# BattleZips/BattleZips-Halo2

Measured on AMD Instinct MI355X. Metric: complete proofs per second (synthesis + create_proof), BoardCircuit, k=14, IPA/Pasta, higher is better.
Workload: dtype u32x8 (255-bit modular integer, Montgomery)

## Files before the change

battlezips-halo2_amd/csrc/ctx.hpp:

```cpp
#pragma once
#include <hip/hip_runtime.h>
#include <sched.h>

#include <algorithm>
#include <cstdint>
#include <cstdlib>
#include <cstring>
#include <mutex>
#include <string>
#include <vector>

#include "../../include/bzh2.h"

struct bzh_bases {
    int curve = 0;
    size_t n = 0;
    uint32_t* d_xy = nullptr;
    int device = 0;
    int pre_c = 0;
    int pre_nwin = 0;
    size_t row_stride = 0;
    size_t vec_col_stride = 0;
    uint32_t* d_xy29 = nullptr;
};
// ... 91 lines not shown
    if ((al & 15) == 0) {
        const size_t n16 = bytes / 16;
        const unsigned blocks = (unsigned)std::min<size_t>((n16 + 255) / 256, 2048);
        hipLaunchKernelGGL(k_xfer16, dim3(blocks), dim3(256), 0, ctx->stream, (uint4*)dst, (const uint4*)src, n16);
    } else if ((al & 3) == 0) {
        const size_t n4 = bytes / 4;
        const unsigned blocks = (unsigned)std::min<size_t>((n4 + 255) / 256, 2048);
        hipLaunchKernelGGL(k_xfer4, dim3(blocks), dim3(256), 0, ctx->stream, (uint32_t*)dst, (const uint32_t*)src, n4);
    } else {
        BZH_HIP_TRY(ctx, hipMemcpyAsync(dst, src, bytes, fallback, ctx->stream));
        return BZH_OK;
    }
    BZH_HIP_TRY(ctx, hipGetLastError());
    return BZH_OK;
}
inline int pin_big_ensure(bzh_ctx* ctx, size_t bytes) {
    if (ctx->pin_big_bytes >= bytes) return BZH_OK;
    BZH_HIP_TRY(ctx, hipStreamSynchronize(ctx->stream));
    for (auto& p : ctx->pending_d2h) memcpy(p.dst, p.slot, p.bytes);
    ctx->pending_d2h.clear();
    if (ctx->pin_big) BZH_HIP_TRY(ctx, hipHostFree(ctx->pin_big));
    ctx->pin_big = nullptr;
    ctx->pin_big_bytes = 0;
    const size_t want = bytes + (bytes >> 2) + 4096;
    BZH_HIP_TRY(ctx, hipHostMalloc((void**)&ctx->pin_big, want, hipHostMallocDefault));
    ctx->pin_big_bytes = want;
    ctx->pin_big_off = 0;
    return BZH_OK;
}
inline int pin_big_take(bzh_ctx* ctx, size_t bytes, char** out) {
// ... 54 lines not shown
    return bytes > ((size_t)1 << 20) ? pin_big_take(ctx, bytes, slot) : pin_ring_take(ctx, bytes, slot);
}
inline int h2d_commit(bzh_ctx* ctx, void* dst, const char* slot, size_t bytes) {
    return xfer_launch(ctx, dst, slot, bytes, hipMemcpyHostToDevice);
}
inline int d2h_async(bzh_ctx* ctx, void* host_dst, const void* dev_src, size_t bytes) {
    if (!bytes) return BZH_OK;
    char* slot = nullptr;
    int rc = bytes > ((size_t)1 << 20) ? pin_big_take(ctx, bytes, &slot) : pin_ring_take(ctx, bytes, &slot);
    if (rc) return rc;
    rc = xfer_launch(ctx, slot, dev_src, bytes, hipMemcpyDeviceToHost);
    if (rc) return rc;
    ctx->pending_d2h.push_back({host_dst, slot, bytes});
    return BZH_OK;
}
inline int d2h_finish(bzh_ctx* ctx) {
    BZH_HIP_TRY(ctx, hipStreamSynchronize(ctx->stream));
    for (auto& p : ctx->pending_d2h) memcpy(p.dst, p.slot, p.bytes);
    ctx->pending_d2h.clear();
    return BZH_OK;
}

struct ScopedTimer {
    bzh_ctx* ctx;
    int cls;
    hipEvent_t a = nullptr, b = nullptr;
    ScopedTimer(bzh_ctx* c, int k) : ctx(c), cls(k) {
        if (!ctx->profiling) return;
        a = take();
        b = take();
// ... 10 lines not shown
            ctx->event_pool.pop_back();
            return e;
        }
        hipEvent_t e = nullptr;
        if (hipEventCreate(&e) != hipSuccess) return nullptr;
        return e;
    }
};

int msm_run(bzh_ctx* ctx, const bzh_bases* bases, const uint32_t* d_scalars, size_t n, size_t batch, int form,
            uint32_t* d_out_xyz);
int msm_run_paired(bzh_ctx* ctx, const bzh_bases* bases, const uint32_t* d_scalars, size_t n_pair, unsigned log_m, size_t batch,
                   int form, uint32_t* d_out_xyz);
int ntt_run(bzh_ctx* ctx, int field, uint32_t* d_data, unsigned log_n, size_t batch, const uint64_t* omega,
            const uint64_t* coset_shift, int inverse, int form);
int ntt_run_padded(bzh_ctx* ctx, int field, uint32_t* d_dst, const uint32_t* d_src, unsigned src_log, unsigned log_n, size_t batch,
                   const uint64_t* omega, const uint64_t* coset_shift, uint32_t* d_out29 = nullptr);
int bases_to_montgomery(bzh_ctx* ctx, int curve, uint32_t* d_xy, size_t n);
int bases_precompute(bzh_ctx* ctx, bzh_bases* bases, int window_bits);
size_t msm_collapse_scratch_bytes(const bzh_bases* srs, size_t cnt, size_t batch, int c_tail);
int msm_collapse_table(bzh_ctx* ctx, const bzh_bases* srs, const uint32_t* d_s, size_t cnt, size_t batch, int c_tail, uint32_t* d_table29, uint32_t* d_table,
                       void* d_scratch, bzh_bases* out);
int field_convert(bzh_ctx* ctx, int field, uint32_t* d, size_t count, int to_mont);
int poly_batch_invert(bzh_ctx* ctx, int field, uint32_t* d, size_t count);
int poly_prefix_product(bzh_ctx* ctx, int field, uint32_t* d, size_t n, size_t batch);
int poly_eval(bzh_ctx* ctx, int field, const uint32_t* coeffs, size_t n, size_t batch, const uint32_t* xs, size_t x_stride,
              uint32_t* out);
int poly_inner_product(bzh_ctx* ctx, int field, const uint32_t* a, const uint32_t* b, size_t n, size_t batch, uint32_t* out);
int poly_fold(bzh_ctx* ctx, int field, const uint32_t* in, size_t half, size_t batch, const uint32_t* u, size_t u_stride,
              uint32_t* out);
// ... 25 lines not shown
```

battlezips-halo2_amd/csrc/ipa.hip:

```cpp
#include <cstring>
#include <vector>

#include "block.cuh"
#include "ctx.hpp"
#include "curve.cuh"
#include "host_field.hpp"

namespace bzh {

template <class P>
__global__ void __launch_bounds__(256) k_reduce_wide(const uint32_t* __restrict__ in, size_t count, uint32_t* __restrict__ out) {
    const size_t g = blockIdx.x * (size_t)blockDim.x + threadIdx.x;
    if (g >= count) return;
    Fe<P> lo = fe_load<P>(in + g * 16), hi = fe_load<P>(in + g * 16 + 8);
    Fe<P> r2 = fe_r2<P>();
    fe_store(out + g * 8, fe_add(fe_mul(lo, r2), fe_mul(fe_mul(hi, r2), r2)));
}

template <class P>
__global__ void __launch_bounds__(256) k_ipa_s_update(const uint32_t* __restrict__ s, size_t count, const uint32_t* __restrict__ u,
                                                        uint32_t* __restrict__ s_new) {
    const size_t g = blockIdx.x * (size_t)blockDim.x + threadIdx.x;
    if (g >= count) return;
    const Fe<P> v = fe_load<P>(s + g * 8);
// ... 212 lines not shown
    const bool paired = bases->pre_c != 0 && k >= 1;
    uint32_t* d_commit = take(B * (n + 2) * 8);
    uint32_t* d_tail_table = jstar ? take(B * (tail_m + 2) * (size_t)tail_nwin * 16) : nullptr;
    uint32_t* d_tail_table29 = jstar ? take(B * (tail_m + 2) * (size_t)tail_nwin * 20) : nullptr;
    void* d_tail_scratch = jstar ? (void*)take((tail_scratch + 3) / 4) : nullptr;
    uint32_t* d_hc = take(B * kHc * 8);
    uint32_t* d_dv = take(B * 8);
    uint32_t* d_vlr = take(B * 2 * 8);
    void* d_out = nullptr;
    BZH_TRY(ws_ensure(ctx, 5, 2 * B * 96, &d_out));

    const unsigned g256 = 256;
    auto grid2 = [&](size_t c) { return dim3((unsigned)((c + g256 - 1) / g256), (unsigned)B); };
    if (B > 65535) return BZH_E_ARG;

    if (d_raw_in) {
        BZH_HIP_TRY(ctx, hipMemcpyAsync(d_raw, d_raw_in, B * nrand * 64, hipMemcpyDeviceToDevice, st));
    } else {
        for (size_t b = 0; b < B; b++)
            BZH_TRY(h2d_small(ctx, d_raw + b * nrand * 16, rng_bytes + b * rng_stride, nrand * 64));
    }
    hipLaunchKernelGGL((k_reduce_wide<SF>), dim3((unsigned)((B * nrand + g256 - 1) / g256)), dim3(g256), 0, st, d_raw, B * nrand,
                       d_rand);
    BZH_HIP_TRY(ctx, hipMemcpy2DAsync(d_spoly, n * 32, d_rand, nrand * 32, n * 32, B, hipMemcpyDeviceToDevice, st));
    std::vector<Fe<SF>> tail(B * ntail);
    for (size_t b = 0; b < B; b++) BZH_TRY(d2h_async(ctx, &tail[b * ntail], d_rand + (b * nrand + n) * 8, ntail * 32));

    std::vector<Fe<SF>> hc(B * kHc, fe_zero<SF>());
    for (size_t b = 0; b < B; b++) hc[b * kHc] = fe_to_mont(fe_from_u64<SF>(x3s + 4 * b));
    auto push_hc = [&]() -> int {
        return h2d_small(ctx, d_hc, hc.data(), B * kHc * 32);
    };
    BZH_TRY(push_hc());
    BZH_TRY(poly_eval(ctx, field, d_spoly, n, B, d_hc, kHc, d_dv));
    hipLaunchKernelGGL((k_sub_at0_batch<SF>), dim3((unsigned)((B + 63) / 64)), dim3(64), 0, st, d_spoly, n, d_dv, B);
    hipLaunchKernelGGL((k_ipa_commit_scalars<SF>), grid2(n + 2), dim3(g256), 0, st, d_spoly, d_rand, n, nrand, d_commit);
    BZH_HIP_TRY(ctx, hipGetLastError());
    BZH_TRY(msm_run(ctx, bases, d_commit, n + 2, B, BZH_FORM_MONTGOMERY, (uint32_t*)d_out));
    std::vector<uint64_t> jac(2 * B * 12), xy(2 * B * 8);
    BZH_TRY(d2h_async(ctx, jac.data(), d_out, B * 96));
    BZH_TRY(d2h_finish(ctx));
// ... 337 lines not shown
```

battlezips-halo2_amd/csrc/ntt.hip:

```cpp
#include <cstdlib>
#include <cstring>
#include <vector>

#include "host_field.hpp"
#include "ntt_common.cuh"

namespace bzh {

template <class P>
void launch_ntt_pass_wave(const NttPassArgs& aa, unsigned tiles, unsigned nb, hipStream_t stream);
extern template void launch_ntt_pass_wave<FpParams>(const NttPassArgs&, unsigned, unsigned, hipStream_t);
extern template void launch_ntt_pass_wave<FqParams>(const NttPassArgs&, unsigned, unsigned, hipStream_t);
extern template void launch_ntt_pass_wave<BnFrParams>(const NttPassArgs&, unsigned, unsigned, hipStream_t);

template <class P, int C, bool FIRST>
__device__ __forceinline__ void stage_group(uint4* tile, const NttPassArgs& g, int s0, int items, int tid) {
    constexpr int E = 1 << C;
    const int r = g.r, logW = g.logW, W = 1 << logW;
    const int ngroups = items >> C;
    const int stride = 1 << (s0 + logW);
    for (int gi = tid; gi < ngroups; gi += kNttThreads) {
        const int col = gi & (W - 1), gg = gi >> logW;
        const int lo = gg & ((1 << s0) - 1), hi = gg >> s0;
        const int base = ((((hi << C) << s0) | lo) << logW) + col;
// ... 263 lines not shown
                wrow = fe_mul(wrow, wa);
            }
            logA += bits[p];
        }
    }
    BZH_HIP_TRY(ctx, hipMalloc((void**)&d.d_tables, words * 4));
    BZH_HIP_TRY(ctx, hipMemcpyAsync(d.d_tables, host.data(), words * 4, hipMemcpyHostToDevice, ctx->stream));
    BZH_HIP_TRY(ctx, hipStreamSynchronize(ctx->stream));
    return BZH_OK;
}

template <class P>
static int ntt_run_t(bzh_ctx* ctx, uint32_t* d_data, unsigned log_n, size_t batch, const uint64_t* omega,
                     const uint64_t* coset_shift, int inverse, int form, const uint32_t* d_src = nullptr, unsigned src_log = 0,
                     uint32_t* d_out29 = nullptr) {
    if (log_n == 0) return d_out29 ? BZH_E_ARG : BZH_OK;
    Fe<P> w, sh = fe_one<P>();
    for (int i = 0; i < 4; i++) {
        w.l[2 * i] = (uint32_t)omega[i];
        w.l[2 * i + 1] = (uint32_t)(omega[i] >> 32);
        if (coset_shift) {
            sh.l[2 * i] = (uint32_t)coset_shift[i];
            sh.l[2 * i + 1] = (uint32_t)(coset_shift[i] >> 32);
        }
    }
    if (form == BZH_FORM_CANONICAL) {
        w = fe_to_mont(w);
        if (coset_shift) sh = fe_to_mont(sh);
    }
    NttCache* cache = cache_for(ctx);
    NttDomain* dom = nullptr;
// ... 17 lines not shown
        cache->doms.push_back(d);
        dom = &cache->doms.back();
    }
    const size_t total = batch << log_n;
    if (form == BZH_FORM_CANONICAL) {
        int rc = field_convert(ctx, P::id, d_data, total, 1);
        if (rc) return rc;
    }
    int bits[5];
    const int np = plan_passes(log_n, bits);
    int nz = 0;
    if (d_src) {
        if (src_log > log_n || form != BZH_FORM_MONTGOMERY) return BZH_E_ARG;
        nz = (int)(log_n - src_log);
        if ((np < 2 || nz > bits[0] || nz == 0) && !d_data) return BZH_E_ARG;
        if (np < 2 || nz > bits[0] || nz == 0) {
            BZH_HIP_TRY(ctx, hipMemsetAsync(d_data, 0, total * 32, ctx->stream));
            BZH_HIP_TRY(ctx, hipMemcpy2DAsync(d_data, ((size_t)32) << log_n, d_src, ((size_t)32) << src_log, ((size_t)32) << src_log, batch,
                                              hipMemcpyDeviceToDevice, ctx->stream));
            nz = 0;
            d_src = nullptr;
        }
    }
    uint32_t* d_scratch = nullptr;
    if (np >= 2) {
        void* sp = nullptr;
        int rc = ws_ensure(ctx, 0, total * 32, &sp);
        if (rc) return rc;
        d_scratch = (uint32_t*)sp;
    }
    const bool pre = (!inverse && coset_shift);
    const bool post = (inverse != 0);
    int logA = 0;
    for (int p = 0; p < np; p++) {
        NttPassArgs a;
        a.src = (p == 0) ? (nz ? d_src : d_data) : d_scratch;
        a.nz = (p == 0) ? nz : 0;
        a.dst = (p == np - 1) ? d_data : d_scratch;
        a.log_n = log_n;
        a.r = bits[p];
        a.logA = logA;
        a.logB = (int)log_n - logA - bits[p];
        a.last = (p == np - 1);
        int logW = 11 - a.r;
        if (!a.last && logW > a.logB) logW = a.logB;
        if (a.last && logW > logA) logW = logA;
        a.logW = logW;
        a.nprev = p;
        for (int q = 0; q < 4; q++) a.prev_bits[q] = q < p ? bits[q] : 0;
        a.sub_tw = dom->d_tables + dom->off_sub[a.r];
        a.tw_lo = dom->d_tables + dom->off_tw_lo;
// ... 68 lines not shown
    if (!count) return BZH_OK;
    dim3 grid((unsigned)((count + 255) / 256)), block(256);
    BZH_TRY(with_field(field, [&](auto p) {
        hipLaunchKernelGGL((k_field_convert<decltype(p)>), grid, block, 0, ctx->stream, d, count, to_mont);
        return BZH_OK;
    }));
    BZH_HIP_TRY(ctx, hipGetLastError());
    return BZH_OK;
}

int ntt_run(bzh_ctx* ctx, int field, uint32_t* d_data, unsigned log_n, size_t batch, const uint64_t* omega,
            const uint64_t* coset_shift, int inverse, int form) {
    return with_field(field, [&](auto p) { return ntt_run_t<decltype(p)>(ctx, d_data, log_n, batch, omega, coset_shift, inverse, form); });
}

int ntt_run_padded(bzh_ctx* ctx, int field, uint32_t* d_dst, const uint32_t* d_src, unsigned src_log, unsigned log_n, size_t batch,
                   const uint64_t* omega, const uint64_t* coset_shift, uint32_t* d_out29) {
    const int f = BZH_FORM_MONTGOMERY;
    if (d_out29 && field != BZH_FIELD_FP && field != BZH_FIELD_FQ) return BZH_E_ARG;
    return with_field(field, [&](auto p) {
        using P = decltype(p);
        if constexpr (fe29_supported<P>())
            return ntt_run_t<P>(ctx, d_dst, log_n, batch, omega, coset_shift, 0, f, d_src, src_log, d_out29);
        else
            return ntt_run_t<P>(ctx, d_dst, log_n, batch, omega, coset_shift, 0, f, d_src, src_log);
    });
}

}
```

battlezips-halo2_amd/csrc/prove_kernels.cuh:

```cuda
#pragma once
namespace bzh {

namespace {

template <class P>
__global__ void __launch_bounds__(256) k_scale_rows(uint32_t* __restrict__ v, size_t n, const uint32_t* __restrict__ s,
                                                      size_t s_stride) {
    const size_t i = blockIdx.x * (size_t)blockDim.x + threadIdx.x, b = blockIdx.y;
    if (i >= n) return;
    uint32_t* e = v + (b * n + i) * 8;
    fe_store(e, fe_mul(fe_load<P>(e), fe_load<P>(s + b * s_stride * 8)));
}

template <class P>
__global__ void __launch_bounds__(256) k_commit_shift(const uint32_t* __restrict__ polys, size_t pitch, size_t n, size_t ref_row,
                                                        const uint32_t* __restrict__ blinds, uint32_t* __restrict__ sc) {
    const size_t i = blockIdx.x * (size_t)blockDim.x + threadIdx.x, v = blockIdx.y;
    if (i >= n + 3) return;
    const Fe<P> c = fe_load<P>(polys + (v * pitch + ref_row) * 8);
    Fe<P> o;
    if (i < n) o = fe_sub(fe_load<P>(polys + (v * pitch + i) * 8), c);
    else if (i == n) o = fe_zero<P>();
    else if (i == n + 1) o = fe_load<P>(blinds + v * 8);
    else o = c;
    fe_store(sc + (v * (n + 3) + i) * 8, o);
}

template <class P>
__global__ void __launch_bounds__(256) k_sat_to_fe29_planes(const uint32_t* __restrict__ src, uint32_t* __restrict__ dst, size_t size) {
    const size_t i = blockIdx.x * (size_t)256 + threadIdx.x, c = blockIdx.y;
    if (i >= size) return;
    fe29_store_planes<P>(dst + c * 9 * size, i, size, fe29_from_sat_reduced(fe_load<P>(src + (c * size + i) * 8)));
}

__global__ void __launch_bounds__(256) k_any_nonzero(const uint32_t* __restrict__ p, size_t words, size_t row_stride_words,
                                                       uint32_t* __restrict__ flag) {
    const size_t i = blockIdx.x * (size_t)blockDim.x + threadIdx.x, b = blockIdx.y;
    if (i < words && p[b * row_stride_words + i]) atomicOr(flag, 1u);
}

// ... 18 lines not shown
```

battlezips-halo2_amd/csrc/prover.hpp:

```cpp
#pragma once
template <class C>
struct Prover {
    using SF = typename CurveInfo<C>::SF;
    using PB = typename C::Base;
    bzh_ctx* ctx;
    bzh_pk& pk;
    const size_t B;
    hipStream_t st;
    const size_t n, en, usable;
    const int field;
    std::vector<bzh_transcript*> T;
    std::vector<const uint8_t*> rng;
    bool seeded = false;
    std::vector<uint32_t> seed_keys;
    uint32_t* d_seed_keys = nullptr;
    uint64_t seed_ctr = 0;
    std::vector<uint64_t> host_ctr;
    std::vector<std::map<int, Fe<SF>>> env;
    Arena& arena;

    Prover(bzh_ctx* c, bzh_pk& p, size_t batch, Arena& ar)
        : ctx(c), pk(p), B(batch), st(c->stream), n(p.n), en(p.en), usable(p.usable), field(p.field), T(batch, nullptr), rng(batch),
          env(batch), arena(ar) {}
    ~Prover() {
// ... 7 lines not shown
        if (!trace) return;
        (void)hipStreamSynchronize(st);
        const auto now = std::chrono::steady_clock::now();
        fprintf(stderr, "[bzh_prove_batch] %-22s %8.2f ms\n", name, std::chrono::duration<double, std::milli>(now - t_last).count());
        t_last = now;
    }

    uint32_t* dalloc(size_t elems) { return (uint32_t*)arena.alloc(elems * 32); }
    const bool q29 = [&] {
        if constexpr (!fe29_supported<SF>()) return false;
        std::lock_guard<std::mutex> lk(pk.mu);
        return pk.q_ok && pk.q_builtin29 && pk.key29 && pk.q_select == BZH_QUOTIENT_BUILTIN && pk.en % 128 == 0 && pk.ek >= 12 &&
               pk.ek <= 27  && !getenv("BZH_QUOTIENT_V1");
    }();
    uint32_t* ext_alloc(size_t cols) { return q29 ? (uint32_t*)arena.alloc(cols * 9 * en * 4) : dalloc(cols * en); }
    int zero(uint32_t* p, size_t elems) {
        BZH_HIP_TRY(ctx, hipMemsetAsync(p, 0, elems * 32, st));
        return BZH_OK;
    }
    int copy2d(uint32_t* dst, size_t dpitch, const uint32_t* src, size_t spitch, size_t width, size_t rows) {
        if (!rows || !width) return BZH_OK;
        BZH_HIP_TRY(ctx, hipMemcpy2DAsync(dst, dpitch * 32, src, spitch * 32, width * 32, rows, hipMemcpyDeviceToDevice, st));
        return BZH_OK;
    }
    int upload(uint32_t* dst, const Fe<SF>* src, size_t elems) { return h2d_small(ctx, dst, src, elems * 32); }
    struct ProgramArgs {
        uint32_t* consts = nullptr;
        char *prog = nullptr, *ptrs = nullptr, *strides = nullptr;
    };
    int upload_program(const void* cv, size_t cv_bytes, const void* ops, size_t op_bytes, const void* ptrs, const void* strides, size_t ncols,
                       ProgramArgs& out) {
        auto al = [](size_t v) { return (v + 255) & ~(size_t)255; };
        const size_t o_prog = al(cv_bytes), o_ptrs = o_prog + al(op_bytes), o_strides = o_ptrs + al(ncols * 8), total = o_strides + al(ncols * 8);
        char* dev = (char*)arena.alloc(total);
        if (!dev) return BZH_E_OOM;
        char* slot = nullptr;
        BZH_TRY(h2d_stage(ctx, total, &slot));
        memcpy(slot, cv, cv_bytes);
// ... 52 lines not shown
        return random_field(ctx, field, raw, B * count, dst);
    }
    Fe<SF> squeeze(size_t b) {
        uint64_t ch[4];
        bzh_transcript_squeeze_challenge(T[b], ch);
        return fe_to_mont(fe_from_u64<SF>(ch));
    }
    void write_scalar(size_t b, const Fe<SF>& v) {
        uint64_t s[4];
        fe_to_u64<SF>(s, fe_from_mont(v));
        bzh_transcript_write_scalar(T[b], s);
    }

    int to_coeff(uint32_t* dst, const uint32_t* src, size_t count) {
        if (!count) return BZH_OK;
        BZH_HIP_TRY(ctx, hipMemcpyAsync(dst, src, count * n * 32, hipMemcpyDeviceToDevice, st));
        return ntt_run(ctx, field, dst, pk.k, count, pk.omega, nullptr, 1, BZH_FORM_MONTGOMERY);
    }
    int to_extended(uint32_t* dst, const uint32_t* polys, size_t count) {
        if (!count) return BZH_OK;
        if (q29) return ntt_run_padded(ctx, field, nullptr, polys, pk.k, pk.ek, count, pk.eomega, pk.zeta, dst);
        return ntt_run_padded(ctx, field, dst, polys, pk.k, pk.ek, count, pk.eomega, pk.zeta);
    }
    int commit(const uint32_t* polys, size_t pitch, size_t count, const std::vector<Fe<SF>>& blinds, std::vector<uint64_t>& xy,
               bool lagrange = false, long shift_row = -1) {
        xy.assign(count * 8, 0);
        if (!count) return BZH_OK;
        ArenaScope scope(arena);
        static const bool no_shift = getenv("BZH_NO_COMMIT_SHIFT") != nullptr;
        const bool wide = lagrange && pk.srs_lagrange->n == n + 3;
        const bool shift = wide && shift_row >= 0 && !no_shift && count <= 65535;
        const size_t cols = wide ? n + 3 : n + 2;
        uint32_t* sc = dalloc(count * cols);
        uint32_t* bl = dalloc(count);
        uint32_t* d_out = dalloc(count * 3);
        if (!sc || !bl || !d_out) return BZH_E_OOM;
        BZH_TRY(upload(bl, blinds.data(), count));
        if (shift) {
            hipLaunchKernelGGL((k_commit_shift<SF>), dim3((unsigned)((n + 3 + 255) / 256), (unsigned)count), dim3(256), 0, st, polys, pitch, n,
                               (size_t)shift_row, bl, sc);
            BZH_HIP_TRY(ctx, hipGetLastError());
        } else {
            BZH_TRY(zero(sc, count * cols));
            BZH_TRY(copy2d(sc, cols, polys, pitch, n, count));
            BZH_TRY(copy2d(sc + (n + 1) * 8, cols, bl, 1, 1, count));
        }
        BZH_TRY(msm_run(ctx, lagrange ? pk.srs_lagrange : pk.srs, sc, cols, count, BZH_FORM_MONTGOMERY, d_out));
        std::vector<uint64_t> jac(count * 12);
        BZH_TRY(d2h_async(ctx, jac.data(), d_out, count * 96));
        BZH_TRY(d2h_finish(ctx));
        h_jac_to_affine<PB>(jac.data(), count, BZH_FORM_MONTGOMERY, BZH_FORM_CANONICAL, xy.data());
        return BZH_OK;
    }
    int evals(const uint32_t* stacked, size_t count, const std::vector<Fe<SF>>& points, std::vector<Fe<SF>>& out) {
        out.resize(count);
        if (!count) return BZH_OK;
        ArenaScope scope(arena);
        uint32_t* xs = dalloc(count);
        uint32_t* res = dalloc(count);
        if (!xs || !res) return BZH_E_OOM;
// ... 174 lines not shown
    const int na = pk.na, nf = pk.nf, ni = pk.ni, bf = pk.bf, nsets = pk.nsets, nl = pk.nl, npieces = pk.npieces;
    const size_t bf1 = (size_t)bf + 1, m = pk.perm_columns.size();
    const int nz = nsets + nl;
    std::vector<uint64_t> xy;
    std::vector<Fe<SF>> blinds;
    for (size_t b = 0; b < B; b++) {
        BZH_TRY(bzh_transcript_new(field, &T[b]));
        bzh_transcript_common_scalar(T[b], pk.vk_repr);
    }

    mark("setup");
    uint32_t* inst = dalloc(B * std::max(ni, 1) * n);
    uint32_t* inst_polys = dalloc(B * std::max(ni, 1) * n);
    if (!inst || !inst_polys) return BZH_E_OOM;
    if (ni) {
        BZH_TRY(zero(inst, B * ni * n));
        if (inst_rows) {
            std::vector<Fe<SF>> hv(B * ni * inst_rows);
            for (size_t i = 0; i < hv.size(); i++) hv[i] = fe_to_mont(fe_from_u64<SF>(instances + 4 * i));
            uint32_t* tmp = dalloc(hv.size());
            if (!tmp) return BZH_E_OOM;
            BZH_TRY(upload(tmp, hv.data(), hv.size()));
            BZH_TRY(copy2d(inst, n, tmp, inst_rows, inst_rows, B * ni));
        }
        BZH_TRY(to_coeff(inst_polys, inst, B * ni));
        blinds.assign(B * ni, fe_one<SF>());
        if (pk.srs_lagrange) BZH_TRY(commit(inst, n, B * ni, blinds, xy, true));
        else BZH_TRY(commit(inst_polys, n, B * ni, blinds, xy));
        for (size_t b = 0; b < B; b++)
            for (int i = 0; i < ni; i++) bzh_transcript_common_point(T[b], &xy[(b * ni + i) * 8]);
    }

    mark("instance");
    uint32_t* adv = dalloc(B * na * n);
    uint32_t* adv_polys = dalloc(B * na * n);
    if (!adv || !adv_polys) return BZH_E_OOM;
    BZH_HIP_TRY(ctx, hipMemcpyAsync(adv, d_advice_in, B * na * n * 32, hipMemcpyDeviceToDevice, st));
    {
        uint32_t* rows = dalloc(B * na * bf1);
        if (!rows) return BZH_E_OOM;
        BZH_TRY(draw_rows(na * bf1, rows));
        BZH_TRY(copy2d(adv + usable * 8, n, rows, bf1, bf1, B * na));
    }
    std::vector<Fe<SF>> adv_blinds(B * na);
    for (size_t b = 0; b < B; b++)
        for (int i = 0; i < na; i++) adv_blinds[b * na + i] = draw(b);
    BZH_TRY(to_coeff(adv_polys, adv, B * na));
    if (pk.srs_lagrange) BZH_TRY(commit(adv, n, B * na, adv_blinds, xy, true));
    else BZH_TRY(commit(adv_polys, n, B * na, adv_blinds, xy));
    for (size_t b = 0; b < B; b++) {
        for (int i = 0; i < na; i++) bzh_transcript_write_point(T[b], C::id, &xy[(b * na + i) * 8]);
        env[b][SY_THETA] = squeeze(b);
// ... 51 lines not shown
                BZH_TRY(lookup_permute(ctx, field, d.a_c, d.s_c, n, usable, B, BZH_FORM_MONTGOMERY, d.as, d.as + n * 8, 2 * n, n, ws, &d_status));
                BZH_TRY(d2h_async(ctx, lk_status.data(), d_status, B * sizeof(int32_t)));
                BZH_TRY(d2h_finish(ctx));
            }
            for (int32_t rc : lk_status)
                if (rc) return rc;
            mark(" lk:permute");
        } else {
            char *ah_c = nullptr, *sh_c = nullptr, *as_c = nullptr;
            BZH_TRY(pin_big_reserve(ctx, 4 * B * n * 32 + ((size_t)3 << 20)));
            BZH_TRY(pin_big_take(ctx, B * n * 32, &ah_c));
            BZH_TRY(pin_big_take(ctx, B * n * 32, &sh_c));
            BZH_TRY(pin_big_take(ctx, B * 2 * n * 32, &as_c));
            uint32_t* canon = dalloc(2 * B * n);
            if (!canon) return BZH_E_OOM;
            BZH_HIP_TRY(ctx, hipMemcpyAsync(canon, d.a_c, B * n * 32, hipMemcpyDeviceToDevice, st));
            BZH_HIP_TRY(ctx, hipMemcpyAsync(canon + B * n * 8, d.s_c, B * n * 32, hipMemcpyDeviceToDevice, st));
            BZH_TRY(field_convert(ctx, field, canon, 2 * B * n, 0));
            BZH_TRY(xfer_launch(ctx, ah_c, canon, B * n * 32, hipMemcpyDeviceToHost));
            BZH_TRY(xfer_launch(ctx, sh_c, canon + B * n * 8, B * n * 32, hipMemcpyDeviceToHost));
            BZH_HIP_TRY(ctx, hipStreamSynchronize(st));
            const uint64_t* ah = (const uint64_t*)ah_c;
            const uint64_t* sh = (const uint64_t*)sh_c;
            mark(" lk:compress+d2h");
            BZH_TRY(extend_witness());
            mark(" lk:extend_witness");
            uint64_t* as = (uint64_t*)as_c;
            for (size_t v = 0; v < 2 * B; v++) memset(as + (v * n + usable) * 4, 0, (n - usable) * 32);
            {
                const size_t nthreads = std::min<size_t>({B, (size_t)host_thread_budget(), (size_t)8});
                std::vector<int> rcs(B, BZH_OK);
                std::vector<std::thread> th;
// ... 176 lines not shown
        int qrc = q29 ? run_quotient29(qp, en, h) : (getenv("BZH_QUOTIENT_V1") ? BZH_E_RANGE : run_quotient(reg, en, h));
        if (qrc == BZH_E_RANGE && !q29) {
            qrc = run(key(40, 0), [&](EPool& ep) {
                int tinv = -1;
                const std::vector<int> terms = quotient_terms<SF>(pk, reg, ep, &tinv);
                return ep.mul(ep.horner(terms, ep.sym(SY_Y)), tinv);
            }, reg, en, h);
        }
        BZH_TRY(qrc);
    }
    BZH_TRY(ntt_run(ctx, field, h, pk.ek, B, pk.eomega, pk.zeta, 1, BZH_FORM_MONTGOMERY));
    uint32_t* d_flag = (uint32_t*)arena.alloc(256);
    if (!d_flag) return BZH_E_OOM;
    uint32_t h_flag = 0;
    if ((size_t)npieces * n < en) {
        BZH_HIP_TRY(ctx, hipMemsetAsync(d_flag, 0, 4, st));
        const size_t words = (en - (size_t)npieces * n) * 8;
        hipLaunchKernelGGL(k_any_nonzero, dim3((unsigned)((words + 255) / 256), (unsigned)B), dim3(256), 0, st,
                           h + (size_t)npieces * n * 8, words, en * 8, d_flag);
        BZH_TRY(d2h_async(ctx, &h_flag, d_flag, 4));
    }
    std::vector<Fe<SF>> h_blinds(B * npieces);
    for (size_t b = 0; b < B; b++)
        for (int i = 0; i < npieces; i++) h_blinds[b * npieces + i] = draw(b);
    {
        uint32_t* pieces = dalloc(B * npieces * n);
        if (!pieces) return BZH_E_OOM;
        BZH_TRY(copy2d(pieces, (size_t)npieces * n, h, en, (size_t)npieces * n, B));
        BZH_TRY(commit(pieces, n, B * npieces, h_blinds, xy));
    }
    if (h_flag) {
// ... 32 lines not shown
        where[key(K_LZ, i)] = {z_polys + (size_t)(nsets + i) * n * 8, (size_t)nz * n};
        where[key(K_LA, i)] = {lk[i].polys, 2 * n};
        where[key(K_LS, i)] = {lk[i].polys + n * 8, 2 * n};
    }
    auto gather = [&](const std::vector<std::pair<const uint32_t*, size_t>>& srcs, uint32_t* dst) -> int {
        const size_t J = srcs.size();
        std::vector<const uint32_t*> ps(J);
        std::vector<size_t> ss(J);
        for (size_t j = 0; j < J; j++) {
            ps[j] = srcs[j].first;
            ss[j] = srcs[j].second;
        }
        char* stage = (char*)arena.alloc(J * 16 + 512);
        if (!stage) return BZH_E_OOM;
        char* d_ss = stage + ((J * 8 + 255) & ~(size_t)255);
        BZH_TRY(h2d_small(ctx, stage, ps.data(), J * 8));
        BZH_TRY(h2d_small(ctx, d_ss, ss.data(), J * 8));
        hipLaunchKernelGGL(k_gather_rows, dim3((unsigned)((2 * n + 255) / 256), (unsigned)J, (unsigned)B), dim3(256), 0, st, (uint4*)dst,
                           (const uint4* const*)stage, (const size_t*)d_ss, n, J);
        BZH_HIP_TRY(ctx, hipGetLastError());
        return BZH_OK;
    };
    {
        std::vector<std::pair<uint64_t, int>> jobs;
        for (auto& a : pk.instance_queries) jobs.push_back({key(K_INST, a.first), a.second});
        for (auto& a : pk.advice_queries) jobs.push_back({key(K_ADV, a.first), a.second});
        for (auto& a : pk.fixed_queries) jobs.push_back({key(K_FIX, a.first), a.second});
        jobs.push_back({key(K_MISC, M_F), 0});
        for (size_t j = 0; j < m; j++) jobs.push_back({key(K_SIGMA, j), 0});
        for (int i = 0; i < nsets; i++) {
            jobs.push_back({key(K_PZ, i), 0});
            jobs.push_back({key(K_PZ, i), 1});
// ... 143 lines not shown
                        num.swap(nx);
                    }
                    const Fe<SF> cf = fe_mul(ev[b * J2 + o2 + j], dinv[b * J2 + o2 + j]);
                    for (size_t i = 0; i < num.size(); i++) res[i] = fe_add(res[i], fe_mul(cf, num[i]));
                }
                for (size_t i = 0; i < np; i++) r_small[(b * nq + si) * maxpts + i] = res[i];
                o2 += np;
            }
        }
        uint32_t* rcols = dalloc(B * nq * n);
        uint32_t* rs_dev = dalloc(B * nq * maxpts);
        uint32_t* f_parts = dalloc(B * nq * n);
        uint32_t* k_a = dalloc(B * nq * n);
        uint32_t* k_b = dalloc(B * nq * n);
        if (!rcols || !rs_dev || !f_parts || !k_a || !k_b) return BZH_E_OOM;
        BZH_TRY(zero(rcols, B * nq * n));
        BZH_TRY(zero(f_parts, B * nq * n));
        BZH_TRY(upload(rs_dev, r_small.data(), r_small.size()));
        BZH_TRY(copy2d(rcols, n, rs_dev, maxpts, maxpts, B * nq));
        std::vector<size_t> order(nq);
        for (size_t si = 0; si < nq; si++) order[si] = si;
        std::stable_sort(order.begin(), order.end(), [&](size_t x, size_t y) { return pk.rot_sets[x].size() > pk.rot_sets[y].size(); });
        const size_t steps = nq ? pk.rot_sets[order[0]].size() : 0;
        size_t nkate = 0;
        for (size_t si = 0; si < nq; si++) nkate += pk.rot_sets[si].size();
        uint32_t* d_xall = dalloc(std::max<size_t>(nkate, 1) * B);
        if (!d_xall) return BZH_E_OOM;
        {
            std::vector<Fe<SF>> xv(nkate * B);
            size_t at = 0;
            for (size_t t = 0; t < steps; t++)
                for (size_t pos = 0; pos < nq && pk.rot_sets[order[pos]].size() > t; pos++)
                    for (size_t b = 0; b < B; b++) xv[at++] = rot(b, pk.rot_sets[order[pos]][t]);
            BZH_TRY(upload(d_xall, xv.data(), xv.size()));
// ... 6 lines not shown
            BZH_TRY(run(key(42, 0), [&](EPool& ep) { return ep.sub(ep.query(0), ep.query(1)); }, reg, n, k_a + pos * B * n * 8));
        }
        {
            uint32_t* cur = k_a;
            uint32_t* nxt = k_b;
            size_t len = n, x_at = 0;
            for (size_t t = 0; t < steps; t++) {
                size_t active = 0;
                while (active < nq && pk.rot_sets[order[active]].size() > t) active++;
                BZH_TRY(poly_kate_division(ctx, field, cur, len, active * B, d_xall + x_at * 8, nxt));
                x_at += active * B;
                std::swap(cur, nxt);
                len--;
                for (size_t pos = 0; pos < active; pos++)
                    if (pk.rot_sets[order[pos]].size() == t + 1)
                        BZH_TRY(copy2d(f_parts + order[pos] * n * 8, nq * n, cur + pos * B * len * 8, len, len, B));
            }
            for (size_t pos = 0; pos < nq; pos++)
                if (pk.rot_sets[order[pos]].empty()) BZH_TRY(copy2d(f_parts + order[pos] * n * 8, nq * n, k_a + pos * B * n * 8, n, n, B));
        }
        mark("multiopen_q_kate");
        uint32_t* f_poly = dalloc(B * n);
        uint32_t* p_poly = dalloc(B * n);
        if (!f_poly || !p_poly) return BZH_E_OOM;
        if (nq == 1) {
            BZH_TRY(copy2d(f_poly, n, f_parts, n, n, B));
        } else {
            Cols reg;
            for (size_t si = 0; si < nq; si++) reg.add(key(K_MISC, M_H0 + si), f_parts + si * n * 8, nq * n);
            BZH_TRY(run(key(43, 0), [&](EPool& ep) {
                std::vector<int> t;
// ... 84 lines not shown
```

Before: 745.6.

## Replace hipMemcpy2D/memset calls with fused copy-pad kernels and batched row staging

Swaps hipMemcpy2DAsync, hipMemsetAsync and device-to-device hipMemcpyAsync for custom kernels, including a copy kernel that zero-pads each row in the same pass, so separate memset-then-copy pairs collapse into one launch. Per-batch host uploads and downloads are grouped into a single staged transfer, the to_coeff copy is folded into an NTT that reads from a separate source, and commit scratch assembly becomes one kernel. The aim is fewer API calls and less redundant memory traffic. The risk is that custom kernels may copy more slowly than the runtime's copy paths, and the NTT source-handling change alters which buffers are read.

```diff
diff --git a/battlezips-halo2_amd/csrc/ctx.hpp b/battlezips-halo2_amd/csrc/ctx.hpp
--- a/battlezips-halo2_amd/csrc/ctx.hpp
+++ b/battlezips-halo2_amd/csrc/ctx.hpp
@@ -129,6 +129,56 @@
     BZH_HIP_TRY(ctx, hipGetLastError());
     return BZH_OK;
 }
+static __global__ void __launch_bounds__(256) k_copy_rows(uint4* __restrict__ dst, size_t dpitch, const uint4* __restrict__ src, size_t spitch,
+                                                          size_t width16, size_t rows) {
+    for (size_t r = blockIdx.y; r < rows; r += gridDim.y)
+        for (size_t i = blockIdx.x * (size_t)256 + threadIdx.x; i < width16; i += (size_t)gridDim.x * 256) dst[r * dpitch + i] = src[r * spitch + i];
+}
+static __global__ void __launch_bounds__(256) k_copy_rows4(uint32_t* __restrict__ dst, size_t dpitch, const uint32_t* __restrict__ src,
+                                                           size_t spitch, size_t width4, size_t rows) {
+    for (size_t r = blockIdx.y; r < rows; r += gridDim.y)
+        for (size_t i = blockIdx.x * (size_t)256 + threadIdx.x; i < width4; i += (size_t)gridDim.x * 256) dst[r * dpitch + i] = src[r * spitch + i];
+}
+static __global__ void __launch_bounds__(256) k_copy_rows_pad(uint4* __restrict__ dst, size_t dpitch, const uint4* __restrict__ src,
+                                                              size_t spitch, size_t width16, size_t total16, size_t rows) {
+    for (size_t r = blockIdx.y; r < rows; r += gridDim.y)
+        for (size_t i = blockIdx.x * (size_t)256 + threadIdx.x; i < total16; i += (size_t)gridDim.x * 256)
+            dst[r * dpitch + i] = i < width16 ? src[r * spitch + i] : make_uint4(0u, 0u, 0u, 0u);
+}
+static __global__ void __launch_bounds__(256) k_fill_zero(uint4* __restrict__ dst, size_t n16) {
+    for (size_t i = blockIdx.x * (size_t)256 + threadIdx.x; i < n16; i += (size_t)gridDim.x * 256) dst[i] = make_uint4(0u, 0u, 0u, 0u);
+}
+inline dim3 rows_grid(size_t words, size_t rows) {
+    return dim3((unsigned)std::min<size_t>((words + 255) / 256, 2048), (unsigned)std::min<size_t>(rows, 65535));
+}
+inline int copy_rows_launch(bzh_ctx* ctx, void* dst, size_t dpitch, const void* src, size_t spitch, size_t row_bytes, size_t rows,
+                            size_t pad_bytes = 0) {
+    if (!rows || (!row_bytes && !pad_bytes)) return BZH_OK;
+    const uintptr_t al = (uintptr_t)dst | (uintptr_t)src | dpitch | spitch | row_bytes | pad_bytes;
+    if (pad_bytes > row_bytes) {
+        if (al & 15) return BZH_E_ARG;
+        hipLaunchKernelGGL(k_copy_rows_pad, rows_grid(pad_bytes / 16, rows), dim3(256), 0, ctx->stream, (uint4*)dst, dpitch / 16, (const uint4*)src,
+                           spitch / 16, row_bytes / 16, pad_bytes / 16, rows);
+    } else if ((al & 15) == 0) {
+        hipLaunchKernelGGL(k_copy_rows, rows_grid(row_bytes / 16, rows), dim3(256), 0, ctx->stream, (uint4*)dst, dpitch / 16, (const uint4*)src,
+                           spitch / 16, row_bytes / 16, rows);
+    } else if ((al & 3) == 0) {
+        hipLaunchKernelGGL(k_copy_rows4, rows_grid(row_bytes / 4, rows), dim3(256), 0, ctx->stream, (uint32_t*)dst, dpitch / 4, (const uint32_t*)src,
+                           spitch / 4, row_bytes / 4, rows);
+    } else {
+        return BZH_E_ARG;
+    }
+    BZH_HIP_TRY(ctx, hipGetLastError());
+    return BZH_OK;
+}
+inline int fill_zero_launch(bzh_ctx* ctx, void* dst, size_t bytes) {
+    if (!bytes) return BZH_OK;
+    if (((uintptr_t)dst | bytes) & 15) return BZH_E_ARG;
+    const size_t n16 = bytes / 16;
+    hipLaunchKernelGGL(k_fill_zero, dim3((unsigned)std::min<size_t>((n16 + 255) / 256, 2048)), dim3(256), 0, ctx->stream, (uint4*)dst, n16);
+    BZH_HIP_TRY(ctx, hipGetLastError());
+    return BZH_OK;
+}
 inline int pin_big_ensure(bzh_ctx* ctx, size_t bytes) {
     if (ctx->pin_big_bytes >= bytes) return BZH_OK;
     BZH_HIP_TRY(ctx, hipStreamSynchronize(ctx->stream));
@@ -213,6 +263,49 @@
     ctx->pending_d2h.push_back({host_dst, slot, bytes});
     return BZH_OK;
 }
+static constexpr size_t kRowsSlotMax = (size_t)128 << 20;
+inline int h2d_rows(bzh_ctx* ctx, void* dev_dst, size_t dev_pitch, const void* host_src, size_t host_pitch, size_t row_bytes, size_t rows) {
+    if (!row_bytes || !rows) return BZH_OK;
+    if (((uintptr_t)dev_dst | dev_pitch | row_bytes) & 3) {
+        for (size_t r = 0; r < rows; r++) {
+            int rc = h2d_small(ctx, (char*)dev_dst + r * dev_pitch, (const char*)host_src + r * host_pitch, row_bytes);
+            if (rc) return rc;
+        }
+        return BZH_OK;
+    }
+    const size_t slot_pitch = (row_bytes + 15) & ~(size_t)15, group = std::max<size_t>(kRowsSlotMax / slot_pitch, 1);
+    for (size_t r0 = 0; r0 < rows; r0 += group) {
+        const size_t nr = std::min(group, rows - r0);
+        char* slot = nullptr;
+        int rc = h2d_stage(ctx, slot_pitch * nr, &slot);
+        if (rc) return rc;
+        for (size_t r = 0; r < nr; r++) memcpy(slot + r * slot_pitch, (const char*)host_src + (r0 + r) * host_pitch, row_bytes);
+        rc = copy_rows_launch(ctx, (char*)dev_dst + r0 * dev_pitch, dev_pitch, slot, slot_pitch, row_bytes, nr);
+        if (rc) return rc;
+    }
+    return BZH_OK;
+}
+inline int d2h_async_rows(bzh_ctx* ctx, void* host_dst, size_t host_pitch, const void* dev_src, size_t dev_pitch, size_t row_bytes, size_t rows) {
+    if (!row_bytes || !rows) return BZH_OK;
+    if (((uintptr_t)dev_src | dev_pitch | row_bytes) & 3) {
+        for (size_t r = 0; r < rows; r++) {
+            int rc = d2h_async(ctx, (char*)host_dst + r * host_pitch, (const char*)dev_src + r * dev_pitch, row_bytes);
+            if (rc) return rc;
+        }
+        return BZH_OK;
+    }
+    const size_t slot_pitch = (row_bytes + 15) & ~(size_t)15, group = std::max<size_t>(kRowsSlotMax / slot_pitch, 1);
+    for (size_t r0 = 0; r0 < rows; r0 += group) {
+        const size_t nr = std::min(group, rows - r0);
+        char* slot = nullptr;
+        int rc = h2d_stage(ctx, slot_pitch * nr, &slot);
+        if (rc) return rc;
+        rc = copy_rows_launch(ctx, slot, slot_pitch, (const char*)dev_src + r0 * dev_pitch, dev_pitch, row_bytes, nr);
+        if (rc) return rc;
+        for (size_t r = 0; r < nr; r++) ctx->pending_d2h.push_back({(char*)host_dst + (r0 + r) * host_pitch, slot + r * slot_pitch, row_bytes});
+    }
+    return BZH_OK;
+}
 inline int d2h_finish(bzh_ctx* ctx) {
     BZH_HIP_TRY(ctx, hipStreamSynchronize(ctx->stream));
     for (auto& p : ctx->pending_d2h) memcpy(p.dst, p.slot, p.bytes);
@@ -253,6 +346,8 @@
                    int form, uint32_t* d_out_xyz);
 int ntt_run(bzh_ctx* ctx, int field, uint32_t* d_data, unsigned log_n, size_t batch, const uint64_t* omega,
             const uint64_t* coset_shift, int inverse, int form);
+int ntt_run_from(bzh_ctx* ctx, int field, uint32_t* d_dst, const uint32_t* d_src, unsigned log_n, size_t batch, const uint64_t* omega,
+                 const uint64_t* coset_shift, int inverse);
 int ntt_run_padded(bzh_ctx* ctx, int field, uint32_t* d_dst, const uint32_t* d_src, unsigned src_log, unsigned log_n, size_t batch,
                    const uint64_t* omega, const uint64_t* coset_shift, uint32_t* d_out29 = nullptr);
 int bases_to_montgomery(bzh_ctx* ctx, int curve, uint32_t* d_xy, size_t n);
diff --git a/battlezips-halo2_amd/csrc/ipa.hip b/battlezips-halo2_amd/csrc/ipa.hip
--- a/battlezips-halo2_amd/csrc/ipa.hip
+++ b/battlezips-halo2_amd/csrc/ipa.hip
@@ -250,17 +250,13 @@
     auto grid2 = [&](size_t c) { return dim3((unsigned)((c + g256 - 1) / g256), (unsigned)B); };
     if (B > 65535) return BZH_E_ARG;
 
-    if (d_raw_in) {
-        BZH_HIP_TRY(ctx, hipMemcpyAsync(d_raw, d_raw_in, B * nrand * 64, hipMemcpyDeviceToDevice, st));
-    } else {
-        for (size_t b = 0; b < B; b++)
-            BZH_TRY(h2d_small(ctx, d_raw + b * nrand * 16, rng_bytes + b * rng_stride, nrand * 64));
-    }
-    hipLaunchKernelGGL((k_reduce_wide<SF>), dim3((unsigned)((B * nrand + g256 - 1) / g256)), dim3(g256), 0, st, d_raw, B * nrand,
-                       d_rand);
-    BZH_HIP_TRY(ctx, hipMemcpy2DAsync(d_spoly, n * 32, d_rand, nrand * 32, n * 32, B, hipMemcpyDeviceToDevice, st));
+    if (!d_raw_in) BZH_TRY(h2d_rows(ctx, d_raw, nrand * 64, rng_bytes, rng_stride, nrand * 64, B));
+    hipLaunchKernelGGL((k_reduce_wide<SF>), dim3((unsigned)((B * nrand + g256 - 1) / g256)), dim3(g256), 0, st, d_raw_in ? d_raw_in : d_raw,
+                       B * nrand, d_rand);
+    BZH_HIP_TRY(ctx, hipGetLastError());
+    BZH_TRY(copy_rows_launch(ctx, d_spoly, n * 32, d_rand, nrand * 32, n * 32, B));
     std::vector<Fe<SF>> tail(B * ntail);
-    for (size_t b = 0; b < B; b++) BZH_TRY(d2h_async(ctx, &tail[b * ntail], d_rand + (b * nrand + n) * 8, ntail * 32));
+    BZH_TRY(d2h_async_rows(ctx, tail.data(), ntail * 32, d_rand + n * 8, nrand * 32, ntail * 32, B));
 
     std::vector<Fe<SF>> hc(B * kHc, fe_zero<SF>());
     for (size_t b = 0; b < B; b++) hc[b * kHc] = fe_to_mont(fe_from_u64<SF>(x3s + 4 * b));
diff --git a/battlezips-halo2_amd/csrc/ntt.hip b/battlezips-halo2_amd/csrc/ntt.hip
--- a/battlezips-halo2_amd/csrc/ntt.hip
+++ b/battlezips-halo2_amd/csrc/ntt.hip
@@ -301,7 +301,10 @@
 static int ntt_run_t(bzh_ctx* ctx, uint32_t* d_data, unsigned log_n, size_t batch, const uint64_t* omega,
                      const uint64_t* coset_shift, int inverse, int form, const uint32_t* d_src = nullptr, unsigned src_log = 0,
                      uint32_t* d_out29 = nullptr) {
-    if (log_n == 0) return d_out29 ? BZH_E_ARG : BZH_OK;
+    if (log_n == 0) {
+        if (d_out29) return BZH_E_ARG;
+        return d_src && d_data ? xfer_launch(ctx, d_data, d_src, batch * 32, hipMemcpyDeviceToDevice) : BZH_OK;
+    }
     Fe<P> w, sh = fe_one<P>();
     for (int i = 0; i < 4; i++) {
         w.l[2 * i] = (uint32_t)omega[i];
@@ -349,10 +352,9 @@
         if (src_log > log_n || form != BZH_FORM_MONTGOMERY) return BZH_E_ARG;
         nz = (int)(log_n - src_log);
         if ((np < 2 || nz > bits[0] || nz == 0) && !d_data) return BZH_E_ARG;
-        if (np < 2 || nz > bits[0] || nz == 0) {
-            BZH_HIP_TRY(ctx, hipMemsetAsync(d_data, 0, total * 32, ctx->stream));
-            BZH_HIP_TRY(ctx, hipMemcpy2DAsync(d_data, ((size_t)32) << log_n, d_src, ((size_t)32) << src_log, ((size_t)32) << src_log, batch,
-                                              hipMemcpyDeviceToDevice, ctx->stream));
+        if (nz && (np < 2 || nz > bits[0])) {
+            BZH_TRY(copy_rows_launch(ctx, d_data, ((size_t)32) << log_n, d_src, ((size_t)32) << src_log, ((size_t)32) << src_log, batch,
+                                     ((size_t)32) << log_n));
             nz = 0;
             d_src = nullptr;
         }
@@ -369,7 +371,7 @@
     int logA = 0;
     for (int p = 0; p < np; p++) {
         NttPassArgs a;
-        a.src = (p == 0) ? (nz ? d_src : d_data) : d_scratch;
+        a.src = (p == 0) ? (d_src ? d_src : d_data) : d_scratch;
         a.nz = (p == 0) ? nz : 0;
         a.dst = (p == np - 1) ? d_data : d_scratch;
         a.log_n = log_n;
@@ -468,6 +470,14 @@
     return with_field(field, [&](auto p) { return ntt_run_t<decltype(p)>(ctx, d_data, log_n, batch, omega, coset_shift, inverse, form); });
 }
 
+int ntt_run_from(bzh_ctx* ctx, int field, uint32_t* d_dst, const uint32_t* d_src, unsigned log_n, size_t batch, const uint64_t* omega,
+                 const uint64_t* coset_shift, int inverse) {
+    if (!d_dst || !d_src) return BZH_E_ARG;
+    return with_field(field, [&](auto p) {
+        return ntt_run_t<decltype(p)>(ctx, d_dst, log_n, batch, omega, coset_shift, inverse, BZH_FORM_MONTGOMERY, d_src, log_n);
+    });
+}
+
 int ntt_run_padded(bzh_ctx* ctx, int field, uint32_t* d_dst, const uint32_t* d_src, unsigned src_log, unsigned log_n, size_t batch,
                    const uint64_t* omega, const uint64_t* coset_shift, uint32_t* d_out29) {
     const int f = BZH_FORM_MONTGOMERY;
diff --git a/battlezips-halo2_amd/csrc/prove_kernels.cuh b/battlezips-halo2_amd/csrc/prove_kernels.cuh
--- a/battlezips-halo2_amd/csrc/prove_kernels.cuh
+++ b/battlezips-halo2_amd/csrc/prove_kernels.cuh
@@ -24,6 +24,18 @@
     else if (i == n + 1) o = fe_load<P>(blinds + v * 8);
     else o = c;
     fe_store(sc + (v * (n + 3) + i) * 8, o);
+}
+
+__global__ void __launch_bounds__(256) k_commit_rows(const uint4* __restrict__ polys, size_t pitch, size_t n, size_t cols,
+                                                       const uint4* __restrict__ blinds, uint4* __restrict__ sc, size_t count) {
+    const size_t i = blockIdx.x * (size_t)blockDim.x + threadIdx.x;
+    if (i >= 2 * cols) return;
+    for (size_t v = blockIdx.y; v < count; v += gridDim.y) {
+        uint4 o = make_uint4(0u, 0u, 0u, 0u);
+        if (i < 2 * n) o = polys[v * pitch * 2 + i];
+        else if (i >= 2 * (n + 1) && i < 2 * (n + 2)) o = blinds[v * 2 + (i - 2 * (n + 1))];
+        sc[v * cols * 2 + i] = o;
+    }
 }
 
 template <class P>
diff --git a/battlezips-halo2_amd/csrc/prover.hpp b/battlezips-halo2_amd/csrc/prover.hpp
--- a/battlezips-halo2_amd/csrc/prover.hpp
+++ b/battlezips-halo2_amd/csrc/prover.hpp
@@ -45,14 +45,9 @@
                pk.ek <= 27  && !getenv("BZH_QUOTIENT_V1");
     }();
     uint32_t* ext_alloc(size_t cols) { return q29 ? (uint32_t*)arena.alloc(cols * 9 * en * 4) : dalloc(cols * en); }
-    int zero(uint32_t* p, size_t elems) {
-        BZH_HIP_TRY(ctx, hipMemsetAsync(p, 0, elems * 32, st));
-        return BZH_OK;
-    }
-    int copy2d(uint32_t* dst, size_t dpitch, const uint32_t* src, size_t spitch, size_t width, size_t rows) {
-        if (!rows || !width) return BZH_OK;
-        BZH_HIP_TRY(ctx, hipMemcpy2DAsync(dst, dpitch * 32, src, spitch * 32, width * 32, rows, hipMemcpyDeviceToDevice, st));
-        return BZH_OK;
+    int zero(uint32_t* p, size_t elems) { return fill_zero_launch(ctx, p, elems * 32); }
+    int copy2d(uint32_t* dst, size_t dpitch, const uint32_t* src, size_t spitch, size_t width, size_t rows, size_t padded = 0) {
+        return copy_rows_launch(ctx, dst, dpitch * 32, src, spitch * 32, width * 32, rows, padded * 32);
     }
     int upload(uint32_t* dst, const Fe<SF>* src, size_t elems) { return h2d_small(ctx, dst, src, elems * 32); }
     struct ProgramArgs {
@@ -135,8 +130,7 @@
 
     int to_coeff(uint32_t* dst, const uint32_t* src, size_t count) {
         if (!count) return BZH_OK;
-        BZH_HIP_TRY(ctx, hipMemcpyAsync(dst, src, count * n * 32, hipMemcpyDeviceToDevice, st));
-        return ntt_run(ctx, field, dst, pk.k, count, pk.omega, nullptr, 1, BZH_FORM_MONTGOMERY);
+        return ntt_run_from(ctx, field, dst, src, pk.k, count, pk.omega, nullptr, 1);
     }
     int to_extended(uint32_t* dst, const uint32_t* polys, size_t count) {
         if (!count) return BZH_OK;
@@ -162,9 +156,9 @@
                                (size_t)shift_row, bl, sc);
             BZH_HIP_TRY(ctx, hipGetLastError());
         } else {
-            BZH_TRY(zero(sc, count * cols));
-            BZH_TRY(copy2d(sc, cols, polys, pitch, n, count));
-            BZH_TRY(copy2d(sc + (n + 1) * 8, cols, bl, 1, 1, count));
+            hipLaunchKernelGGL(k_commit_rows, dim3((unsigned)((2 * cols + 255) / 256), (unsigned)std::min<size_t>(count, 65535)), dim3(256), 0, st,
+                               (const uint4*)polys, pitch, n, cols, (const uint4*)bl, (uint4*)sc, count);
+            BZH_HIP_TRY(ctx, hipGetLastError());
         }
         BZH_TRY(msm_run(ctx, lagrange ? pk.srs_lagrange : pk.srs, sc, cols, count, BZH_FORM_MONTGOMERY, d_out));
         std::vector<uint64_t> jac(count * 12);
@@ -369,14 +363,15 @@
     uint32_t* inst_polys = dalloc(B * std::max(ni, 1) * n);
     if (!inst || !inst_polys) return BZH_E_OOM;
     if (ni) {
-        BZH_TRY(zero(inst, B * ni * n));
         if (inst_rows) {
             std::vector<Fe<SF>> hv(B * ni * inst_rows);
             for (size_t i = 0; i < hv.size(); i++) hv[i] = fe_to_mont(fe_from_u64<SF>(instances + 4 * i));
             uint32_t* tmp = dalloc(hv.size());
             if (!tmp) return BZH_E_OOM;
             BZH_TRY(upload(tmp, hv.data(), hv.size()));
-            BZH_TRY(copy2d(inst, n, tmp, inst_rows, inst_rows, B * ni));
+            BZH_TRY(copy2d(inst, n, tmp, inst_rows, inst_rows, B * ni, n));
+        } else {
+            BZH_TRY(zero(inst, B * ni * n));
         }
         BZH_TRY(to_coeff(inst_polys, inst, B * ni));
         blinds.assign(B * ni, fe_one<SF>());
@@ -390,7 +385,7 @@
     uint32_t* adv = dalloc(B * na * n);
     uint32_t* adv_polys = dalloc(B * na * n);
     if (!adv || !adv_polys) return BZH_E_OOM;
-    BZH_HIP_TRY(ctx, hipMemcpyAsync(adv, d_advice_in, B * na * n * 32, hipMemcpyDeviceToDevice, st));
+    BZH_TRY(xfer_launch(ctx, adv, d_advice_in, B * na * n * 32, hipMemcpyDeviceToDevice));
     {
         uint32_t* rows = dalloc(B * na * bf1);
         if (!rows) return BZH_E_OOM;
@@ -472,8 +467,8 @@
             BZH_TRY(pin_big_take(ctx, B * 2 * n * 32, &as_c));
             uint32_t* canon = dalloc(2 * B * n);
             if (!canon) return BZH_E_OOM;
-            BZH_HIP_TRY(ctx, hipMemcpyAsync(canon, d.a_c, B * n * 32, hipMemcpyDeviceToDevice, st));
-            BZH_HIP_TRY(ctx, hipMemcpyAsync(canon + B * n * 8, d.s_c, B * n * 32, hipMemcpyDeviceToDevice, st));
+            BZH_TRY(xfer_launch(ctx, canon, d.a_c, B * n * 32, hipMemcpyDeviceToDevice));
+            BZH_TRY(xfer_launch(ctx, canon + B * n * 8, d.s_c, B * n * 32, hipMemcpyDeviceToDevice));
             BZH_TRY(field_convert(ctx, field, canon, 2 * B * n, 0));
             BZH_TRY(xfer_launch(ctx, ah_c, canon, B * n * 32, hipMemcpyDeviceToHost));
             BZH_TRY(xfer_launch(ctx, sh_c, canon + B * n * 8, B * n * 32, hipMemcpyDeviceToHost));
@@ -680,7 +675,7 @@
     if (!d_flag) return BZH_E_OOM;
     uint32_t h_flag = 0;
     if ((size_t)npieces * n < en) {
-        BZH_HIP_TRY(ctx, hipMemsetAsync(d_flag, 0, 4, st));
+        BZH_TRY(fill_zero_launch(ctx, d_flag, 16));
         const size_t words = (en - (size_t)npieces * n) * 8;
         hipLaunchKernelGGL(k_any_nonzero, dim3((unsigned)((words + 255) / 256), (unsigned)B), dim3(256), 0, st,
                            h + (size_t)npieces * n * 8, words, en * 8, d_flag);
@@ -743,8 +738,12 @@
         char* stage = (char*)arena.alloc(J * 16 + 512);
         if (!stage) return BZH_E_OOM;
         char* d_ss = stage + ((J * 8 + 255) & ~(size_t)255);
-        BZH_TRY(h2d_small(ctx, stage, ps.data(), J * 8));
-        BZH_TRY(h2d_small(ctx, d_ss, ss.data(), J * 8));
+        char* slot = nullptr;
+        const size_t o_ss = (size_t)(d_ss - stage), up = (o_ss + J * 8 + 15) & ~(size_t)15;
+        BZH_TRY(h2d_stage(ctx, up, &slot));
+        memcpy(slot, ps.data(), J * 8);
+        memcpy(slot + o_ss, ss.data(), J * 8);
+        BZH_TRY(h2d_commit(ctx, stage, slot, up));
         hipLaunchKernelGGL(k_gather_rows, dim3((unsigned)((2 * n + 255) / 256), (unsigned)J, (unsigned)B), dim3(256), 0, st, (uint4*)dst,
                            (const uint4* const*)stage, (const size_t*)d_ss, n, J);
         BZH_HIP_TRY(ctx, hipGetLastError());
@@ -918,10 +917,8 @@
         uint32_t* k_a = dalloc(B * nq * n);
         uint32_t* k_b = dalloc(B * nq * n);
         if (!rcols || !rs_dev || !f_parts || !k_a || !k_b) return BZH_E_OOM;
-        BZH_TRY(zero(rcols, B * nq * n));
-        BZH_TRY(zero(f_parts, B * nq * n));
         BZH_TRY(upload(rs_dev, r_small.data(), r_small.size()));
-        BZH_TRY(copy2d(rcols, n, rs_dev, maxpts, maxpts, B * nq));
+        BZH_TRY(copy2d(rcols, n, rs_dev, maxpts, maxpts, B * nq, n));
         std::vector<size_t> order(nq);
         for (size_t si = 0; si < nq; si++) order[si] = si;
         std::stable_sort(order.begin(), order.end(), [&](size_t x, size_t y) { return pk.rot_sets[x].size() > pk.rot_sets[y].size(); });
@@ -958,7 +955,7 @@
                 len--;
                 for (size_t pos = 0; pos < active; pos++)
                     if (pk.rot_sets[order[pos]].size() == t + 1)
-                        BZH_TRY(copy2d(f_parts + order[pos] * n * 8, nq * n, cur + pos * B * len * 8, len, len, B));
+                        BZH_TRY(copy2d(f_parts + order[pos] * n * 8, nq * n, cur + pos * B * len * 8, len, len, B, n));
             }
             for (size_t pos = 0; pos < nq; pos++)
                 if (pk.rot_sets[order[pos]].empty()) BZH_TRY(copy2d(f_parts + order[pos] * n * 8, nq * n, k_a + pos * B * n * 8, n, n, B));
```

Measured after the change: 748.3, median of 6. No clear change (+0.4%).
